# bertaveira/mojosplat

Measured on AMD Instinct MI355X. Metric: frames/sec at 1M Gaussians 1920x1080 fwd; achieved HBM GB/s vs peak, higher is better.
Workload: dtype f32

## Files before the change

### mojosplat_amd/csrc/binning.hip

```cpp
#include <hip/hip_fp16.h>
#include <stdlib.h>
#include <string.h>

#include <algorithm>
#include <atomic>
#include <mutex>
#include <type_traits>
#include <vector>

#include "project_device.hpp"

#ifdef MS_DIAG
__device__ unsigned long long *g_diag_bin = nullptr;
#define MS_BIN_STAMP(k, j) do { if (g_diag_bin && threadIdx.x == 0 && blockIdx.x < 1024) g_diag_bin[((k) * 1024 + blockIdx.x) * 8 + (j)] = __builtin_amdgcn_s_memrealtime(); } while (0)
#else
#define MS_BIN_STAMP(k, j) do { } while (0)
#endif

namespace {

#ifndef MS_CHUNK
#define MS_CHUNK 2048
#endif
#ifndef MS_PH_WAVES
#define MS_PH_WAVES 8
#endif
constexpr int kHistThreads = 1024;
#ifndef MS_CLAIM_GROUPS
#define MS_CLAIM_GROUPS 4
#endif
constexpr int kClaimGroups = MS_CLAIM_GROUPS;
constexpr int kClaimShift = kClaimGroups == 8 ? 0 : kClaimGroups == 4 ? 1 : kClaimGroups == 2 ? 2 : 3;
static_assert(kClaimGroups == 8 || kClaimGroups == 4 || kClaimGroups == 2 || kClaimGroups == 1, "claim groups: a power of two <= 8");
constexpr int kMaxG = 512;
constexpr int kSmallCapDecl = 1024, kMediumCapDecl = 8192, kLargeCapDecl = 16384;
constexpr int kCoopThreshold = 32;
constexpr int kBandCull = 32;
constexpr int kLightBucket = 32;
constexpr int kLightCap = 256;
constexpr int kLean = 64;
constexpr int kDeferTotal = 128;
static_assert(kLean == ms::kTightLean && kDeferTotal == ms::kTightDeferTotal, "internal flag bits out of sync");
constexpr size_t kMaxLds = 160 * 1024 - 4096;

struct Grid {
    int ts, tw, th, row_begin, row_end;
    int pack, cw, ch;
};

struct LeanRec {
    uint32_t xy0, xy1, depth_bits, n_edges;
};
struct Lean12 {
    uint32_t box, depth_bits, mask32;
};

__device__ __forceinline__ unsigned long long reach_mask(float mx, float my, float ca, float cb, float cc,
                                                        float opacity, int x0, int x1, int y0, int y1, int ts) {
    const int w = x1 - x0, h = y1 - y0;
    const float det = ca * cc - cb * cb;
    if (w * h > 64 || w * h <= 1 || !(det > 0.f) || !(ca > 0.f) || !(cc > 0.f) || !(opacity >= ms::kAlphaThreshold))
        return ~0ull;
    const float s2 = 2.0f * (__logf(opacity * 255.0f) * 1.0001f + 1e-4f);
    const float inv_det = __builtin_amdgcn_rcpf(det), inv_ca = __builtin_amdgcn_rcpf(ca);
    const float Y = __builtin_amdgcn_sqrtf(ca * s2 * inv_det);
    const float dy_right = -(cb * __builtin_amdgcn_rcpf(cc)) * __builtin_amdgcn_sqrtf(cc * s2 * inv_det);
    const float fts = (float)ts, span = (float)(ts - 1), inv_ts = __builtin_amdgcn_rcpf(fts);
    unsigned long long mask = 0;
    for (int r = 0; r < h; ++r) {
        const float yl = (float)((y0 + r) * ts) + 0.5f - my, yh = yl + span;
        const float lo = fmaxf(yl, -Y), hi = fminf(yh, Y);
        if (lo > hi + 0.01f) continue;
        const float dyr = fminf(fmaxf(dy_right, lo), hi), dyl = fminf(fmaxf(-dy_right, lo), hi);
        const float xmax = (-cb * dyr + __builtin_amdgcn_sqrtf(fmaxf(ca * s2 - det * dyr * dyr, 0.f))) * inv_ca + 0.01f;
        const float xmin = (-cb * dyl - __builtin_amdgcn_sqrtf(fmaxf(ca * s2 - det * dyl * dyl, 0.f))) * inv_ca - 0.01f;
        const float base = 0.5f - mx;
        int ta = (int)ceilf((xmin - base - span) * inv_ts - 1e-3f), tb = (int)floorf((xmax - base) * inv_ts + 1e-3f);
        ta = max(ta, x0); tb = min(tb, x1 - 1);
        if (ta > tb) continue;
        const unsigned long long rowbits = (tb - ta + 1 >= 64) ? ~0ull : ((1ull << (tb - ta + 1)) - 1ull);
        mask |= rowbits << (r * w + (ta - x0));
    }
    return mask;
}

__device__ __forceinline__ int chunk_of_block(int b, int G) {
    const int n8 = G >> 3, rem = G & 7, x = b & 7, k = b >> 3;
    return x * n8 + min(x, rem) + k;
}

#ifndef MS_DEAL
#define MS_DEAL 64
#endif
#ifndef MS_PH_TICKETS
#define MS_PH_TICKETS 1
#endif
constexpr int kDeal = MS_DEAL;
static_assert(kDeal >= 64 && kDeal <= 1024 && (kDeal & (kDeal - 1)) == 0, "a slice is a power-of-two number of waves");
struct Deal {
    int64_t n, first, stride;
    int iters;
    __device__ __forceinline__ Deal(int64_t n_pos, int wg, int G) {
        constexpr int kWavesPerSlice = kDeal / 64, kParts = kHistThreads / kDeal;
        const int w = __builtin_amdgcn_readfirstlane((int)(threadIdx.x >> 6));
        const int part = w / kWavesPerSlice, v = w - part * kWavesPerSlice;
        n = n_pos;
        first = ((int64_t)part * G + wg) * kDeal + (int64_t)v * 64;
        stride = (int64_t)kParts * G * kDeal;
        iters = (int)((n_pos + stride - 1) / stride);
    }
    __device__ __forceinline__ int64_t base(int it) const { return first + (int64_t)it * stride; }
};

__device__ __forceinline__ int clampi(float v, int lo, int hi) {
    if (!(v > (float)lo)) return lo;
    if (v >= (float)hi) return hi;
    return (int)v;
}

__device__ __forceinline__ bool tile_bbox(float2 m, int2 r, const Grid &g, int &x0, int &x1,
                                          int &y0, int &y1) {
    const float fts = (float)g.ts;
    float trx, try_, tx, ty;
    if ((g.ts & (g.ts - 1)) == 0) {
        const float inv = 1.0f / fts;
        trx = (float)r.x * inv; try_ = (float)r.y * inv;
        tx = m.x * inv; ty = m.y * inv;
    } else {
        trx = (float)r.x / fts; try_ = (float)r.y / fts;
        tx = m.x / fts; ty = m.y / fts;
    }
    x0 = clampi(floorf(tx - trx), 0, g.tw);
    x1 = clampi(ceilf(tx + trx), 0, g.tw);
    y0 = clampi(floorf(ty - try_), 0, g.th);
    y1 = clampi(ceilf(ty + try_), 0, g.th);
    const bool on_grid = x1 > x0 && y1 > y0;
    y0 = max(y0, g.row_begin);
    y1 = min(y1, g.row_end);
    y1 = max(y1, y0);
    return on_grid;
}

__device__ __forceinline__ void count_on_grid(bool on_grid, unsigned int *s_on_grid) {
    const unsigned long long b = __ballot(on_grid);
    if ((threadIdx.x & 63) == 0 && b) atomicAdd(s_on_grid, (unsigned int)__popcll(b));
}

template <bool PACK>
__device__ __forceinline__ bool bin_box(float2 m, int2 r, const Grid &g, int &x0, int &x1, int &y0, int &y1,
                                        int &edges) {
    edges = 0;
    if constexpr (!PACK) return tile_bbox(m, r, g, x0, x1, y0, y1);
    const Grid gc{g.ts >> 1, g.cw, g.ch, 0, g.ch, 0, 0, 0};
    int cx0, cx1, cy0, cy1;
    const bool on = tile_bbox(m, r, gc, cx0, cx1, cy0, cy1);
    x0 = cx0 >> 1; x1 = (cx1 + 1) >> 1;
    y0 = cy0 >> 1; y1 = (cy1 + 1) >> 1;
    if (!on) { x1 = x0; y1 = y0; }
    y0 = max(y0, g.row_begin);
    y1 = min(y1, g.row_end);
    y1 = max(y1, y0);
    edges = (cx0 > 2 * x0 ? 1 : 0) | (cx1 < 2 * x1 ? 2 : 0) | (cy0 > 2 * y0 ? 4 : 0) | (cy1 < 2 * y1 ? 8 : 0);
    return on;
}

__device__ __forceinline__ int edge_blocks(int edges, int c, int r, int w, int h) {
    int q = 0xf;
    if ((edges & 1) && c == 0) q &= 0xa;
    if ((edges & 2) && c == w - 1) q &= 0x5;
    if ((edges & 4) && r == 0) q &= 0xc;
    if ((edges & 8) && r == h - 1) q &= 0x3;
    return q;
}

__device__ __forceinline__ unsigned long long clip_cells(unsigned long long m, int edges, int w, int h) {
    const int cwid = 2 * w, rows = 2 * h;
    if (cwid * rows < 64) m &= (1ull << (cwid * rows)) - 1ull;
    if (edges & 4) m &= ~((1ull << cwid) - 1ull);
    if (edges & 8) m &= (1ull << ((rows - 1) * cwid)) - 1ull;
    if (edges & 3) {
        unsigned long long p = 1ull;
        for (int sh = cwid; sh < 64; sh <<= 1) p |= p << sh;
        if (edges & 1) m &= ~p;
        if (edges & 2) m &= ~(p << (cwid - 1));
    }
    return m;
}

struct BigQ {
    uint32_t *ent;
    unsigned int *count;
    unsigned int cap;
};

template <bool PACK, bool PAYLOAD, class F>
__device__ __forceinline__ void walk_boxes_impl(int gi, int x0, int x1, int y0, int y1, int n, int edges,
                                                const Grid &g, unsigned long long mask, F &&f, uint32_t payload,
                                                const BigQ *Q = nullptr) {
    auto call = [&](int t, int64_t i, int q, uint32_t pl) __attribute__((always_inline)) {
        if constexpr (PAYLOAD) f(t, i, q, pl);
        else f(t, i, q);
    };
    const int lane = threadIdx.x & 63;
    const int64_t i = gi;
    const bool big = n > kCoopThreshold;
    if (n > 0 && !big) {
        const int w = x1 - x0;
        const float inv_w = __builtin_amdgcn_rcpf((float)w);
        unsigned int m;
        const bool cells = PACK && n <= 16;
        if (cells) {
            const int cw = 2 * w, h = y1 - y0;
            const unsigned int rowmask = cw >= 32 ? 0xffffffffu : ((1u << cw) - 1u);
            m = 0;
            for (int r = 0; r < h; ++r) {
                unsigned int t = ((unsigned int)(mask >> (2 * r * cw)) | (unsigned int)(mask >> ((2 * r + 1) * cw))) & rowmask;
                t = (t | (t >> 1)) & 0x55555555u;
                t = (t | (t >> 1)) & 0x33333333u;
                t = (t | (t >> 2)) & 0x0f0f0f0fu;
                t = (t | (t >> 4)) & 0x00ff00ffu;
                t = (t | (t >> 8)) & 0x0000ffffu;
                m |= t << (r * w);
            }
        } else {
            m = (unsigned int)mask & (n >= 32 ? 0xffffffffu : ((1u << n) - 1u));
        }
        while (m) {
            const int k = __ffs((int)m) - 1;
            m &= m - 1;
            const int r = (int)(((float)k + 0.5f) * inv_w);
            const int c = k - r * w;
            int q;
            if (cells) {
                const int cw = 2 * w, b00 = 2 * r * cw + 2 * c;
                q = (int)((mask >> b00) & 3ull) | ((int)((mask >> (b00 + cw)) & 3ull) << 2);
            } else {
                q = PACK ? edge_blocks(edges, c, r, w, y1 - y0) : 0xf;
            }
            call((y0 + r - g.row_begin) * g.tw + x0 + c, i, q, payload);
        }
    }
    bool queued = false;
    if (Q && Q->cap && big) {
        const unsigned int slot = atomicAdd(Q->count, 1u);
        if (slot < Q->cap) {
            uint32_t *e = Q->ent + 8u * slot;
            e[0] = (uint32_t)x0 | ((uint32_t)y0 << 16); e[1] = (uint32_t)x1 | ((uint32_t)y1 << 16);
            e[2] = (uint32_t)gi; e[3] = payload;
            e[4] = (uint32_t)mask; e[5] = (uint32_t)(mask >> 32); e[6] = (uint32_t)edges;
            queued = true;
        }
    }
    unsigned long long bigmask = __ballot(big && !queued);
    while (bigmask) {
        const int src = __ffsll((long long)bigmask) - 1;
        bigmask &= bigmask - 1;
        const int bx0 = __builtin_amdgcn_readlane(x0, src), bx1 = __builtin_amdgcn_readlane(x1, src);
        const int by0 = __builtin_amdgcn_readlane(y0, src), by1 = __builtin_amdgcn_readlane(y1, src);
        const unsigned long long bm = ((unsigned long long)(unsigned)__builtin_amdgcn_readlane((int)(mask >> 32), src) << 32) |
                                      (unsigned)__builtin_amdgcn_readlane((int)(mask & 0xffffffffu), src);
        const int be = PACK ? __builtin_amdgcn_readlane(edges, src) : 0;
        const int64_t bi = __builtin_amdgcn_readlane(gi, src);
        const uint32_t bp = PAYLOAD ? (uint32_t)__builtin_amdgcn_readlane((int)payload, src) : 0u;
        const int w = bx1 - bx0, cnt = w * (by1 - by0);
        if (w <= 256 && cnt <= 65536) {
            const float inv_w = __builtin_amdgcn_rcpf((float)w);
            for (int k = lane; k < cnt; k += 64) {
                const int r = (int)(((float)k + 0.5f) * inv_w), c = k - r * w;
                if (cnt > 64 || ((bm >> k) & 1ull))
                    call((by0 + r - g.row_begin) * g.tw + bx0 + c, bi, PACK ? edge_blocks(be, c, r, w, by1 - by0) : 0xf, bp);
            }
        } else {
            for (int k = lane; k < cnt; k += 64) {
                const int r = k / w, c = k % w;
                call((by0 + r - g.row_begin) * g.tw + bx0 + c, bi, PACK ? edge_blocks(be, c, r, w, by1 - by0) : 0xf, bp);
            }
        }
    }
}

template <bool PACK, class F>
__device__ __forceinline__ void walk_boxes(int gi, int x0, int x1, int y0, int y1, int n, int edges,
                                           const Grid &g, unsigned long long mask, F &&f, const BigQ *Q = nullptr) {
    walk_boxes_impl<PACK, false>(gi, x0, x1, y0, y1, n, edges, g, mask, f, 0u, Q);
}
template <bool PACK, class F>
__device__ __forceinline__ void walk_boxes(int gi, int x0, int x1, int y0, int y1, int n, int edges,
                                           const Grid &g, unsigned long long mask, F &&f, uint32_t payload, const BigQ *Q = nullptr) {
    walk_boxes_impl<PACK, true>(gi, x0, x1, y0, y1, n, edges, g, mask, f, payload, Q);
}

template <bool PACK, bool PAYLOAD, class F>
__device__ __forceinline__ void drain_big_boxes(const BigQ &Q, const Grid &g, F &&f) {
    if (!Q.cap) return;
    __syncthreads();
    const unsigned int total = min(*Q.count, Q.cap);
    const int lane = threadIdx.x & 63;
    const unsigned int nw = blockDim.x >> 6;
    for (unsigned int e = (unsigned int)__builtin_amdgcn_readfirstlane((int)(threadIdx.x >> 6)); e < total; e += nw) {
        const uint32_t *q = Q.ent + 8u * e;
        const int bx0 = (int)(q[0] & 0xffffu), by0 = (int)(q[0] >> 16), bx1 = (int)(q[1] & 0xffffu), by1 = (int)(q[1] >> 16);
        const int64_t bi = (int64_t)(int32_t)q[2];
        const uint32_t bp = q[3];
        const unsigned long long bm = (unsigned long long)q[4] | ((unsigned long long)q[5] << 32);
        const int be = (int)q[6];
        const int w = bx1 - bx0, cnt = w * (by1 - by0);
        const float inv_w = __builtin_amdgcn_rcpf((float)max(w, 1));
        const bool by_rcp = w <= 256 && cnt <= 65536;
        for (int k = lane; k < cnt; k += 64) {
            const int r = by_rcp ? (int)(((float)k + 0.5f) * inv_w) : k / w, c = k - r * w;
            if (cnt > 64 || ((bm >> k) & 1ull)) {
                const int t = (by0 + r - g.row_begin) * g.tw + bx0 + c;
                const int qb = PACK ? edge_blocks(be, c, r, w, by1 - by0) : 0xf;
// ... 584 lines not shown
        const int t = tb + lane;
        unsigned int incl = c;
#pragma unroll
        for (int d = 1; d < 64; d <<= 1) {
            const unsigned int o = (unsigned int)__shfl_up((int)incl, d);
            if (lane >= d) incl += o;
        }
        if (t < w1) {
            const unsigned long long b = run + (incl - c), e = run + incl;
            reinterpret_cast<int2 *>(tile_ranges)[t] =
                make_int2((int32_t)min(b, 0x7fffffffull), (int32_t)min(e, 0x7fffffffull));
            redo_flag[t] = 0;
            lmax = max(lmax, c);
            if (c > (unsigned)kLargeCapDecl) xl_list[atomicAdd(&s_nxl, 1u)] = t;
            else if (c > (unsigned)kMediumCapDecl) large_list[atomicAdd(&s_nlarge, 1u)] = t;
            else if (c > (unsigned)kSmallCapDecl) medium_list[atomicAdd(&s_nmedium, 1u)] = t;
            if (order && t >= band0 && t < band1) atomicAdd(&s_bkt[bucket_of(c)], 1u);
        }
        run += (unsigned long long)__shfl((int)incl, 63);
    };
#pragma unroll
    for (int k = 0; k < kPre; ++k)
        if (w0 + k * 64 < w1) step(w0 + k * 64, pre[k]);
    for (int tb = w0 + kPre * 64; tb < w1; tb += 64) step(tb, count_of(tb + lane));
#pragma unroll
    for (int d = 32; d > 0; d >>= 1) lmax = max(lmax, (unsigned int)__shfl_xor((int)lmax, d));
    if (lane == 0) atomicMax(&s_max, lmax);
    __syncthreads();
    if (order) {
        if (w == 0) {
            const unsigned int c0 = s_bkt[127 - 2 * lane], c1 = s_bkt[126 - 2 * lane];
            unsigned int incl = c0 + c1;
#pragma unroll
            for (int d = 1; d < 64; d <<= 1) {
                const unsigned int o = (unsigned int)__shfl_up((int)incl, d);
                if (lane >= d) incl += o;
            }
            const unsigned int excl = incl - (c0 + c1);
            s_base[127 - 2 * lane] = excl;
            s_base[126 - 2 * lane] = excl + c0;
        }
        __syncthreads();
        if (threadIdx.x == 0 && A.wg_on_grid) const_cast<uint32_t *>(A.wg_on_grid)[kMaxG + 1] = s_base[kLightBucket];
        __syncthreads();
        auto place = [&](int t, unsigned int c) {
            if (t < w1 && t >= band0 && t < band1) order[atomicAdd(&s_base[bucket_of(c)], 1u)] = t;
        };
#pragma unroll
        for (int k = 0; k < kPre; ++k)
            if (w0 + k * 64 < w1) place(w0 + k * 64 + lane, pre[k]);
        for (int tb = w0 + kPre * 64; tb < w1; tb += 64) place(tb + lane, count_of(tb + lane));
    }
    if (threadIdx.x == 0) {
        info[0] = (int64_t)grand;
        info[1] = (int64_t)s_max;
        info[2] = (int64_t)s_nmedium;
        info[3] = (int64_t)s_nlarge;
        info[4] = (int64_t)s_nxl;
        {
            const int prev_cut = min(max(redo_count[1], 0), max(prev_redo, 0));
            info[5] = (int64_t)(prev_redo - prev_cut) + ((int64_t)(prev_cut & 0x3fffffff) << 32) + (prev_cut > 0 && info[10] != 0 ? (1ll << 62) : 0);
        }
        redo_count[0] = 0;
        redo_count[1] = 0;
        redo_count[2] = redo_signature(g);
        info[6] = (int64_t)s_on_grid;
        info[7] = 0;
        if (info_mirror) {
#pragma unroll
            for (int k = 0; k < 7; ++k) info_mirror[k] = info[k];
            __threadfence_system();
        }
    }
}

template <int kScanTiles>
__global__ __launch_bounds__(1024) void k_tile_scan_wg(int G, int T_local,
                                                       uint32_t *__restrict__ hist,
                                                       uint32_t *__restrict__ tile_count, ScanTotalArgs A) {
    constexpr int kScanSlices = 1024 / kScanTiles;
    __shared__ uint32_t s_part[16][kScanTiles];
    __shared__ int s_last;
    MS_BIN_STAMP(1, 0);
    const int lane = threadIdx.x & 63, w = threadIdx.x >> 6;
    const int tl = threadIdx.x & (kScanTiles - 1), sl = threadIdx.x / kScanTiles;
    const int t = blockIdx.x * kScanTiles + tl;
    constexpr int kRows = kMaxG / kScanSlices;
    const int per = (G + kScanSlices - 1) / kScanSlices;
    const int g0 = sl * per, g1 = min(G, g0 + per);
    uint32_t v[kRows];
    uint32_t sum = 0;
#pragma unroll
    for (int k = 0; k < kRows; ++k) {
        const int gg = g0 + k;
        v[k] = (k < per && gg < g1 && t < T_local) ? hist[(size_t)gg * T_local + t] : 0u;
        sum += v[k];
    }
    uint32_t incl = sum;
#pragma unroll
    for (int d = kScanTiles; d < 64; d <<= 1) {
        const uint32_t o = (uint32_t)__shfl_up((int)incl, d);
        if (lane >= d) incl += o;
    }
    if (lane >= 64 - kScanTiles) s_part[w][tl] = incl;
    MS_BIN_STAMP(1, 1);
    __syncthreads();
    MS_BIN_STAMP(1, 2);
    uint32_t run = incl - sum, total = 0;
#pragma unroll
    for (int ww = 0; ww < 16; ++ww) {
        const uint32_t p = s_part[ww][tl];
        if (ww < w) run += p;
        total += p;
    }
#pragma unroll
    for (int k = 0; k < kRows; ++k) {
        const int gg = g0 + k;
        if (k < per && gg < g1 && t < T_local) {
            hist[(size_t)gg * T_local + t] = run;
            run += v[k];
        }
    }
    if (!A.ticket) {
        if (sl == 0 && t < T_local) tile_count[t] = total;
        MS_BIN_STAMP(1, 3);
        return;
    }
    if (sl == 0 && t < T_local) __hip_atomic_store(&tile_count[t], total, __ATOMIC_RELAXED, __HIP_MEMORY_SCOPE_AGENT);
    asm volatile("s_waitcnt vmcnt(0)" ::: "memory");
    __builtin_amdgcn_fence(__ATOMIC_RELEASE, "workgroup");
    __syncthreads();
    if (threadIdx.x == 0) s_last = __hip_atomic_fetch_add(A.ticket, 1u, __ATOMIC_RELAXED, __HIP_MEMORY_SCOPE_AGENT) == gridDim.x - 1 ? 1 : 0;
    __syncthreads();
    if (!s_last) return;
    tile_scan_total<true>(A);
}

__global__ __launch_bounds__(1024) void k_tile_scan_total(ScanTotalArgs A) { tile_scan_total<false>(A); }

__device__ __forceinline__ unsigned long long tile_prefix_lds(const uint32_t *__restrict__ count, int T, uint32_t *s,
                                                              const uint32_t *__restrict__ add = nullptr,
                                                              const uint32_t *__restrict__ xtot = nullptr, int x_mine = 0) {
    __shared__ unsigned long long s_wtot[16];
    const int tid = threadIdx.x, lane = tid & 63, w = tid >> 6;
    const int per = (T + kHistThreads - 1) / kHistThreads;
    const int j0 = min(T, tid * per), j1 = min(T, j0 + per);
    uint32_t addv[4] = {0u, 0u, 0u, 0u};
    const bool pre = add && per <= 4;
    auto add_of = [&](int j) __attribute__((always_inline)) -> uint32_t {
        uint32_t v = add[j];
        if (xtot)
            for (int x = 0; x < x_mine; ++x) v += xtot[(size_t)x * T + j];
        return v;
    };
    if (pre) {
#pragma unroll
        for (int k = 0; k < 4; ++k)
            if (j0 + k < j1) addv[k] = add_of(j0 + k);
    }
    if (xtot) {
        for (int t = tid; t < T; t += kHistThreads) {
            uint32_t c = 0;
#pragma unroll
            for (int x = 0; x < kClaimGroups; ++x) c += xtot[(size_t)x * T + t];
            s[t] = c;
        }
    } else
    for (int t = tid; t < T; t += kHistThreads) s[t] = count[t];
    __syncthreads();
    unsigned long long sum = 0;
    for (int j = j0; j < j1; ++j) sum += s[j];
    unsigned long long incl = sum;
#pragma unroll
    for (int d = 1; d < 64; d <<= 1) {
        const unsigned long long o = __shfl_up(incl, d);
        if (lane >= d) incl += o;
    }
    if (lane == 63) s_wtot[w] = incl;
    __syncthreads();
    unsigned long long run = incl - sum, grand = 0;
#pragma unroll
    for (int ww = 0; ww < 16; ++ww) {
        if (ww < w) run += s_wtot[ww];
        grand += s_wtot[ww];
    }
    if (pre) {
#pragma unroll
        for (int k = 0; k < 4; ++k)
            if (j0 + k < j1) {
                const uint32_t v = s[j0 + k];
                s[j0 + k] = (uint32_t)min(run, 0x7fffffffull) + addv[k];
                run += v;
            }
    } else {
        for (int j = j0; j < j1; ++j) {
            const uint32_t v = s[j];
            s[j] = (uint32_t)min(run, 0x7fffffffull) + (add ? add_of(j) : 0u);
            run += v;
        }
    }
    __syncthreads();
    return grand;
}

__device__ __forceinline__ void deferred_total(int which, const ScanTotalArgs &A, uint32_t *s, int T_local) {
    const Grid &g = A.g;
    const int band0 = g.row_begin * g.tw, band1 = g.row_end * g.tw;
    const int tid = threadIdx.x, lane = tid & 63;
    if (which == 1) {
        if (!A.order) return;
        __shared__ unsigned int s_bkt[128], s_base[128];
        auto bucket_of = [](unsigned int c) -> int {
            if (c == 0) return 0;
            const int l = 31 - __clz((int)c);
            const int frac = l >= 2 ? (int)((c >> (l - 2)) & 3u) : (int)((c << (2 - l)) & 3u);
            return 1 + 4 * l + frac;
        };
        if (tid < 128) s_bkt[tid] = 0;
        __syncthreads();
        for (int t = tid; t < T_local; t += kHistThreads) atomicAdd(&s_bkt[bucket_of(tile_count_of(A, t, T_local))], 1u);
        __syncthreads();
        if (tid < 64) {
            const unsigned int c0 = s_bkt[127 - 2 * lane], c1 = s_bkt[126 - 2 * lane];
            unsigned int incl = c0 + c1;
#pragma unroll
            for (int d = 1; d < 64; d <<= 1) {
                const unsigned int o = (unsigned int)__shfl_up((int)incl, d);
                if (lane >= d) incl += o;
            }
            const unsigned int excl = incl - (c0 + c1);
            s_base[127 - 2 * lane] = excl;
            s_base[126 - 2 * lane] = excl + c0;
        }
        __syncthreads();
        if (tid == 0 && A.wg_on_grid) const_cast<uint32_t *>(A.wg_on_grid)[kMaxG + 1] = s_base[kLightBucket];
        __syncthreads();
        for (int t = tid; t < T_local; t += kHistThreads)
            A.order[atomicAdd(&s_base[bucket_of(tile_count_of(A, t, T_local))], 1u)] = band0 + t;
        return;
    }
    if (A.far_zero)
        for (int t = tid; t < 2 * A.g.tw * A.g.th; t += kHistThreads) A.far_zero[t] = 0u;
    __shared__ unsigned int s_nmedium, s_nlarge, s_nxl, s_max, s_on_grid, s_far;
    if (tid == 0) { s_nmedium = 0; s_nlarge = 0; s_nxl = 0; s_max = 0; s_on_grid = 0; s_far = 0; }
    const int prev_redo = (tid == 0 && A.redo_count[2] == redo_signature(A.g)) ? *A.redo_count : 0;
    unsigned int on_grid_part = tid < A.G ? A.wg_on_grid[tid] : 0u;
    unsigned int far_part = (A.wg_far && tid < A.G) ? A.wg_far[tid] : 0u;
    const unsigned long long grand = tile_prefix_lds(A.tile_count, T_local, s, nullptr, A.xtot);
    if (tid == 0) s[T_local] = (uint32_t)min(grand, 0x7fffffffull);
    __syncthreads();
#pragma unroll
    for (int d = 32; d > 0; d >>= 1) {
        on_grid_part += (unsigned int)__shfl_xor((int)on_grid_part, d);
        far_part += (unsigned int)__shfl_xor((int)far_part, d);
    }
    if (lane == 0 && on_grid_part) atomicAdd(&s_on_grid, on_grid_part);
    if (lane == 0 && far_part) atomicAdd(&s_far, far_part);
    unsigned int lmax = 0;
    for (int t = tid; t < T_local; t += kHistThreads) {
        const uint32_t b = s[t], e = s[t + 1], c = e - b;
        const int at = band0 + t;
        reinterpret_cast<int2 *>(A.tile_ranges)[at] = make_int2((int32_t)b, (int32_t)e);
        A.redo_flag[at] = 0;
        if (A.xtot) const_cast<uint32_t *>(A.tile_count)[t] = c;
        lmax = max(lmax, c);
        if (c > (unsigned)kLargeCapDecl) A.xl_list[atomicAdd(&s_nxl, 1u)] = at;
        else if (c > (unsigned)kMediumCapDecl) A.large_list[atomicAdd(&s_nlarge, 1u)] = at;
        else if (c > (unsigned)kSmallCapDecl) A.medium_list[atomicAdd(&s_nmedium, 1u)] = at;
    }
    if (!A.band_only) {
        const int32_t m = (int32_t)min(grand, 0x7fffffffull);
        for (int t = tid; t < g.tw * g.th; t += kHistThreads)
            if (t < band0 || t >= band1) {
                reinterpret_cast<int2 *>(A.tile_ranges)[t] = t < band0 ? make_int2(0, 0) : make_int2(m, m);
                A.redo_flag[t] = 0;
            }
    }
#pragma unroll
    for (int d = 32; d > 0; d >>= 1) lmax = max(lmax, (unsigned int)__shfl_xor((int)lmax, d));
    if (lane == 0) atomicMax(&s_max, lmax);
    __syncthreads();
    if (tid == 0) {
        const int prev_cut = min(max(A.redo_count[1], 0), max(prev_redo, 0));
        int64_t rec[7] = {(int64_t)grand + (int64_t)s_far, (int64_t)s_max, (int64_t)s_nmedium, (int64_t)s_nlarge, (int64_t)s_nxl,
                          (int64_t)(prev_redo - prev_cut) + ((int64_t)(prev_cut & 0x3fffffff) << 32) +
                              (prev_cut > 0 && A.info[10] != 0 ? (1ll << 62) : 0), (int64_t)s_on_grid};
#pragma unroll
        for (int k = 0; k < 7; ++k) A.info[k] = rec[k];
        A.info[7] = 0;
        A.info[8] = (int64_t)grand;
        A.info[9] = (int64_t)s_far;
        A.info[10] = 0;
        A.redo_count[0] = 0;
        A.redo_count[1] = 0;
        A.redo_count[2] = redo_signature(A.g);
        if (A.info_mirror) {
#pragma unroll
            for (int k = 0; k < 7; ++k) A.info_mirror[k] = rec[k];
            __threadfence_system();
        }
    }
}

#ifndef MS_SCATTER_WAVES
#define MS_SCATTER_WAVES 8
#endif
template <bool PACK, int LEAN, bool DEFER>
__global__ __launch_bounds__(kHistThreads, (LEAN == 2 ? MS_SCATTER_WAVES : 4)) void k_isect_scatter(
    int64_t N, const float *__restrict__ means2d, const int32_t *__restrict__ radii,
    const float *__restrict__ depths, const unsigned long long *__restrict__ masks,
    const LeanRec *__restrict__ lean, Grid g, int64_t chunk, const uint32_t *__restrict__ hist,
    const int32_t *__restrict__ tile_ranges, int64_t M, uint64_t *__restrict__ keys,
    uint32_t *__restrict__ wg_depth, Candidates cand, int G, ScanTotalArgs A, unsigned int big_q_off, unsigned int big_q_cap) {
    extern __shared__ uint32_t s_cur[];
    const int T_local = (g.row_end - g.row_begin) * g.tw;
    const int band0 = g.row_begin * g.tw;
    __shared__ unsigned int s_big_n;
    if (threadIdx.x == 0) s_big_n = 0;
    const BigQ bigq{reinterpret_cast<uint32_t *>(reinterpret_cast<char *>(s_cur) + big_q_off), &s_big_n, big_q_cap};
    MS_BIN_STAMP(2, 0);
    if constexpr (DEFER) {
        if ((int)blockIdx.x >= G) {
            deferred_total((int)blockIdx.x - G, A, s_cur, T_local);
            MS_BIN_STAMP(2, 4);
            return;
        }
    }
    const int wg = chunk_of_block(blockIdx.x, G);
    const uint32_t *row = hist + (size_t)wg * T_local;
    (void)chunk;
    int64_t n_pos = N;
    if constexpr (LEAN != 0) {
        if (cand.ids) {
            __shared__ uint32_t s_pref[kMaxG + 1];
            CandMap map{s_pref};
            map.build(cand);
            n_pos = (int64_t)s_pref[cand.n_segs];
        }
    }
    const Deal deal(n_pos, wg, G);
    constexpr int kAhead = 4;
    LeanRec r_q[kAhead], r_nx[kAhead];
    unsigned long long m_q[kAhead], m_nx[kAhead];
#pragma unroll
    for (int k = 0; k < kAhead; ++k) { r_q[k] = r_nx[k] = LeanRec{0u, 0u, 0u, 0u}; m_q[k] = m_nx[k] = ~0ull; }
    bool cut = false;
    if constexpr (LEAN == 2 && DEFER) cut = A.cut_stamp != 0u;
    int n_trips = deal.iters;
    int64_t cut_i0 = 0, cut_i1 = 0;
    if (cut) {
        cut_i0 = (int64_t)wg * A.near_cap;
        cut_i1 = cut_i0 + (int64_t)A.wg_far[kMaxG + wg];
        n_trips = (int)((cut_i1 - cut_i0 + kHistThreads - 1) / kHistThreads);
    }
    auto pos_of = [&](int it) __attribute__((always_inline)) -> int64_t {
        if (it >= n_trips) return -1;
        if (cut) {
            const int64_t j = cut_i0 + (int64_t)it * kHistThreads + threadIdx.x;
            return j < cut_i1 ? j : -1;
        }
        const int64_t j = deal.base(it) + (threadIdx.x & 63);
        return j < n_pos ? j : -1;
    };
    auto load_rec = [&](int64_t j, LeanRec &r, unsigned long long &m) __attribute__((always_inline)) {
        if constexpr (LEAN == 2) {
            if (cut) {
                r = A.near_recs[j];
            } else {
                const uint32_t *q = reinterpret_cast<const uint32_t *>(reinterpret_cast<const Lean12 *>(lean) + j);
                r.xy0 = q[0];
                r.xy1 = (uint32_t)j;
                r.depth_bits = q[1];
                r.n_edges = q[2];
            }
        } else {
            r = lean[j];
            if (masks) m = masks[j];
        }
    };
    auto unpack_rec = [&](LeanRec &r, unsigned long long &m, int64_t &gauss) __attribute__((always_inline)) {
        if constexpr (LEAN == 2) {
            const uint32_t box = r.xy0, mk = r.n_edges;
            gauss = (int64_t)r.xy1;
            const uint32_t x0 = box & 0xffu, y0 = (box >> 8) & 0xffu, w = (box >> 16) & 0xffu, h = box >> 24;
            r.xy0 = x0 | (y0 << 16);
            r.xy1 = (x0 + w) | ((y0 + h) << 16);
            r.n_edges = w * h;
            m = w * h > 32u ? ~0ull : (unsigned long long)mk;
        }
    };
    if constexpr (LEAN != 0) {
#pragma unroll
        for (int k = 0; k < kAhead; ++k) {
            const int64_t j = pos_of(k);
            if (j >= 0) load_rec(j, r_nx[k], m_nx[k]);
        }
    }
    MS_BIN_STAMP(2, 1);
    uint32_t *s_tau = s_cur + T_local + 4;
    if (cut)
        for (int t = threadIdx.x; t < T_local; t += kHistThreads) s_tau[t] = A.tau[band0 + t];
    if constexpr (DEFER) {
        (void)tile_prefix_lds(A.tile_count, T_local, s_cur, row, A.xtot, (int)(blockIdx.x & 7) >> kClaimShift);
        MS_BIN_STAMP(2, 2);
    } else {
        for (int t = threadIdx.x; t < T_local; t += kHistThreads) {
            uint32_t c = (uint32_t)tile_ranges[2 * (band0 + t)] + row[t];
            if (A.xtot)
                for (int x = 0; x < ((int)(blockIdx.x & 7) >> kClaimShift); ++x) c += A.xtot[(size_t)x * T_local + t];
            s_cur[t] = c;
        }
        __syncthreads();
    }
    uint32_t dmin = 0xffffffffu, dmax = 0u;
    if constexpr (LEAN != 0) {
        auto emit = [&](int t, int64_t i, int q, uint32_t db) __attribute__((always_inline)) {
            const uint32_t low = PACK ? (((uint32_t)i << 4) | (uint32_t)q) : (uint32_t)i;
            const uint64_t key = ((uint64_t)db << 32) | low;
            const uint32_t slot = atomicAdd(&s_cur[t], 1u);
            if ((int64_t)slot < M) keys[slot] = key;
        };
        auto emit_cut = [&](int t, int64_t i, int q, uint32_t db) __attribute__((always_inline)) { if (db <= s_tau[t]) emit(t, i, q, db); };
        for (int it0 = 0; it0 < n_trips; it0 += kAhead) {
#pragma unroll
            for (int k = 0; k < kAhead; ++k) { r_q[k] = r_nx[k]; m_q[k] = m_nx[k]; }
            if (it0 + kAhead < n_trips) {
#pragma unroll
                for (int k = 0; k < kAhead; ++k) {
                    const int64_t jn = pos_of(it0 + kAhead + k);
                    if (jn >= 0) load_rec(jn, r_nx[k], m_nx[k]);
                }
            }
#pragma unroll
            for (int k = 0; k < kAhead; ++k) {
                if (it0 + k >= n_trips) break;
                LeanRec r = r_q[k];
                unsigned long long mk = m_q[k];
                const int64_t j = pos_of(it0 + k);
                int64_t gi = j;
                unpack_rec(r, mk, gi);
                int x0 = 0, x1 = 0, y0 = 0, y1 = 0, n = 0, edges = 0;
                unsigned long long mask = ~0ull;
                if (j >= 0) {
                    n = (int)(r.n_edges & 0x0fffffffu);
                    edges = (int)(r.n_edges >> 28);
                    x0 = (int)(r.xy0 & 0xffffu); y0 = (int)(r.xy0 >> 16);
                    x1 = (int)(r.xy1 & 0xffffu); y1 = (int)(r.xy1 >> 16);
                    if (masks && (n > 1 || (PACK && n > 0) || cut)) mask = mk;
                }
                const uint32_t dbits = r.depth_bits;
                if (n > 0) { dmin = min(dmin, dbits); dmax = max(dmax, dbits); }
                if constexpr (!PACK) {
                    const int w = x1 - x0;
                    const float inv_w = __builtin_amdgcn_rcpf((float)max(w, 1));
                    unsigned int m = (n > 0 && n <= kCoopThreshold) ? ((unsigned int)mask & (n >= 32 ? 0xffffffffu : ((1u << n) - 1u))) : 0u;
                    const uint64_t key = ((uint64_t)dbits << 32) | (uint32_t)gi;
                    while (m) {
                        int tt[4];
                        bool vv[4];
                        uint32_t slot[4];
#pragma unroll
                        for (int u = 0; u < 4; ++u) {
                            vv[u] = m != 0u;
                            const int k = vv[u] ? __ffs((int)m) - 1 : 0;
                            m &= m - 1u;
                            const int r = (int)(((float)k + 0.5f) * inv_w);
                            tt[u] = (y0 + r - g.row_begin) * g.tw + x0 + (k - r * w);
                        }
#pragma unroll
                        for (int u = 0; u < 4; ++u)
                            if (vv[u]) slot[u] = atomicAdd(&s_cur[tt[u]], 1u);
#pragma unroll
                        for (int u = 0; u < 4; ++u)
                            if (vv[u] && (int64_t)slot[u] < M) keys[slot[u]] = key;
                    }
                    if (cut)
                        walk_boxes<PACK>((int)gi, x0, x1, y0, y1, n > kCoopThreshold ? n : 0, edges, g, mask, emit_cut, dbits, &bigq);
                    else
                        walk_boxes<PACK>((int)gi, x0, x1, y0, y1, n > kCoopThreshold ? n : 0, edges, g, mask, emit, dbits, &bigq);
                } else {
                    walk_boxes<PACK>((int)gi, x0, x1, y0, y1, n, edges, g, mask, emit, dbits, &bigq);
                }
            }
        }
        if (cut) drain_big_boxes<PACK, true>(bigq, g, emit_cut);
        else drain_big_boxes<PACK, true>(bigq, g, emit);
    } else {
        for_each_isect<PACK>(0, N, means2d, radii, masks, g, nullptr, nullptr, cand, G, [&](int t, int64_t i, int q) {
            const uint32_t slot = atomicAdd(&s_cur[t], 1u);
            const uint32_t low = PACK ? (((uint32_t)i << 4) | (uint32_t)q) : (uint32_t)i;
            const uint32_t dbits = __float_as_uint(depths[i]);
            dmin = min(dmin, dbits);
            dmax = max(dmax, dbits);
            const uint64_t key = ((uint64_t)dbits << 32) | low;
            if ((int64_t)slot < M) keys[slot] = key;
        });
    }
    MS_BIN_STAMP(2, 3);
#ifdef MS_DIAG
    if constexpr (LEAN != 0) { __syncthreads(); MS_BIN_STAMP(2, 4); }
#endif
    if (wg_depth) {
        uint32_t *s_depth = s_cur + T_local + 1;
        __syncthreads();
        if (threadIdx.x == 0) { s_depth[0] = 0xffffffffu; s_depth[1] = 0u; }
        __syncthreads();
#pragma unroll
        for (int d = 32; d > 0; d >>= 1) {
            dmin = min(dmin, (uint32_t)__shfl_xor((int)dmin, d));
            dmax = max(dmax, (uint32_t)__shfl_xor((int)dmax, d));
        }
        if ((threadIdx.x & 63) == 0) { atomicMin(&s_depth[0], dmin); atomicMax(&s_depth[1], dmax); }
        __syncthreads();
        if (threadIdx.x == 0) { wg_depth[2 * blockIdx.x] = s_depth[0]; wg_depth[2 * blockIdx.x + 1] = s_depth[1]; }
    }
}

}
#include "sort_device.hpp"
namespace {

constexpr int kSmallCap = SortCfg<256, 4>::CAP;
constexpr int kMediumCap = SortCfg<1024, 8>::CAP;
constexpr int kLargeCap = SortCfg<1024, 16>::CAP;

template <bool SPLIT>
__global__ __launch_bounds__(256) void k_tile_sort_small(const int32_t *__restrict__ tile_ranges,
                                                         const uint64_t *__restrict__ keys,
                                                         int32_t *__restrict__ flatten_ids,
                                                         int64_t *__restrict__ isect_ids, int64_t cap,
                                                         int tile_lo, ms::BlockLists blocks, int bin_w) {
    __shared__ __attribute__((aligned(16))) unsigned char smem[SortCfg<256, 4>::LDS];
    const int tile = tile_lo + blockIdx.x;
    const int start = tile_ranges[2 * tile], n = tile_ranges[2 * tile + 1] - start;
    const bool skip = n <= 0 || (int64_t)start + n > cap;
    if (SPLIT && (skip || n > kSmallCap)) {
        if (threadIdx.x < 4) {
            const int by = tile / bin_w, bx = tile - by * bin_w;
            const int x = 2 * bx + (threadIdx.x & 1), y = 2 * by + (threadIdx.x >> 1);
            if (x < blocks.tw16 && y < blocks.th16)
                reinterpret_cast<int2 *>(blocks.block_ranges)[y * blocks.tw16 + x] = make_int2(0, 0);
        }
        if (threadIdx.x == 0) blocks.bin_more[tile] = 0;
    }
    if (skip || n > kSmallCap) return;
    sort_segment_lds<256, 4>(smem, keys, start, n, tile, flatten_ids, isect_ids, nullptr, SPLIT ? &blocks : nullptr,
                             bin_w);
}

template <int E>
__global__ __launch_bounds__(1024, (E <= 8 ? 8 : 4)) void k_tile_sort_list(const int32_t *__restrict__ list,
                                                         const int32_t *__restrict__ tile_ranges,
                                                         const uint64_t *__restrict__ keys,
                                                         int32_t *__restrict__ flatten_ids,
                                                         int64_t *__restrict__ isect_ids,
                                                         const int64_t *__restrict__ n_list_dev,
                                                         int n_list_host, int64_t cap) {
    extern __shared__ __attribute__((aligned(16))) unsigned char smem_dyn[];
    const int n_list = n_list_dev ? (int)*n_list_dev : n_list_host;
    for (int li = blockIdx.x; li < n_list; li += gridDim.x) {
        const int tile = list[li];
        const int start = tile_ranges[2 * tile], n = tile_ranges[2 * tile + 1] - start;
        if ((int64_t)start + n <= cap)
            sort_segment_lds<1024, E>(smem_dyn, keys, start, n, tile, flatten_ids, isect_ids, nullptr);
        __syncthreads();
    }
}

#ifndef MS_MERGED_WAVES
#define MS_MERGED_WAVES 6
#endif
constexpr int kFrontThreads = 512;
static_assert(kFrontNB == 4 * kFrontThreads, "four buckets per thread in the scan");
constexpr size_t kFrontLds = (size_t)kFrontCap * 8 + (size_t)kFrontNB * 4 + 64 * 4 + 16;

template <bool SPLIT, bool MERGED>
__global__ __launch_bounds__(kFrontThreads, (MERGED ? MS_MERGED_WAVES : 1)) void k_tile_front(const int32_t *__restrict__ medium,
                                                     const int32_t *__restrict__ large,
                                                     const int32_t *__restrict__ xl,
                                                     const int64_t *__restrict__ info_dev, int nm_host, int nl_host,
                                                     int nx_host, const int32_t *__restrict__ tile_ranges,
                                                     const uint64_t *__restrict__ keys,
                                                     int32_t *__restrict__ flatten_ids,
                                                     int32_t *__restrict__ front_count, int64_t cap,
                                                     uint32_t fixed_min, int fixed_shift, int front_k,
                                                     ms::BlockLists blocks, int bin_w,
                                                     const uint32_t *__restrict__ wg_depth, int n_wg,
                                                     const int32_t *__restrict__ order, int n_order, int front_cap,
                                                     const uint32_t *__restrict__ n_big_dev,
                                                     uint32_t *__restrict__ tau, const uint32_t *__restrict__ tau_now,
                                                     const uint32_t *__restrict__ has_far, uint32_t cut_stamp) {
    static_assert(!(SPLIT && MERGED), "block lists are cut by the two-launch path");
    auto next_cut_whole = [&](int tile) {
        if (tau) tau[tile] = (cut_stamp && has_far[tile] == cut_stamp) ? tau_now[tile] : 0xffffffffu;
    };
    extern __shared__ __attribute__((aligned(16))) unsigned char smem_dyn[];
    uint64_t *s_out = reinterpret_cast<uint64_t *>(smem_dyn);
    uint32_t *s_cnt = reinterpret_cast<uint32_t *>(s_out + front_cap);
    uint32_t *s_red = s_cnt + kFrontNB;
    int *s_sel = reinterpret_cast<int *>(s_red + 64);
    constexpr int THREADS = kFrontThreads, NW = kFrontThreads / 64;
    const int tid = threadIdx.x, lane = tid & 63, w = tid >> 6;
    const int nm = info_dev ? (int)info_dev[2] : nm_host, nl = info_dev ? (int)info_dev[3] : nl_host;
    const int nx = info_dev ? (int)info_dev[4] : nx_host;
    const int total = MERGED ? n_order : nm + nl + nx;
    if ((int)blockIdx.x >= total) return;
    const int n_big = (MERGED && n_big_dev) ? min((int)*n_big_dev, total) : -1;
    if constexpr (MERGED) {
        if (n_big >= 0 && (int)blockIdx.x >= n_big) {
            const int e = n_big + 8 * ((int)blockIdx.x - n_big) + w;
            if (e < total) {
                const int tile = order[e];
                const int start = tile_ranges[2 * tile], n = tile_ranges[2 * tile + 1] - start;
                if (n > 0 && n <= kLightCap && (int64_t)start + n <= cap)
                    sort_segment_lds<64, kLightCap / 64>(smem_dyn + (size_t)w * SortCfg<64, kLightCap / 64>::LDS, keys, start, n, tile,
                                                         flatten_ids, nullptr, nullptr);
                if (lane == 0) next_cut_whole(tile);
            }
            return;
        }
    }
#ifdef MS_DIAG
    if (g_diag_bin && tid == 0) g_diag_bin[(3 * 1024 + (blockIdx.x & 1023)) * 8 + (blockIdx.x >> 10) * 3] = __builtin_amdgcn_s_memrealtime();
#endif
    bool range_known = false;
    auto frame_range = [&]() {
      if (wg_depth && !range_known) {
        uint32_t lo = 0xffffffffu, hi = 0u;
        for (int j = tid; j < n_wg; j += THREADS) {
            lo = min(lo, wg_depth[2 * j]);
            hi = max(hi, wg_depth[2 * j + 1]);
        }
#pragma unroll
        for (int d = 32; d > 0; d >>= 1) {
            lo = min(lo, (uint32_t)__shfl_xor((int)lo, d));
            hi = max(hi, (uint32_t)__shfl_xor((int)hi, d));
        }
        if (lane == 0) { s_red[w] = lo; s_red[16 + w] = hi; }
        __syncthreads();
#pragma unroll
        for (int ww = 0; ww < NW; ++ww) { lo = min(lo, s_red[ww]); hi = max(hi, s_red[16 + ww]); }
        __syncthreads();
        if (hi >= lo) {
            const uint32_t span = hi - lo;
            const int bits = span ? 32 - __clz(span) : 0;
            fixed_min = lo;
            fixed_shift = max(0, bits - kFrontLogNB);
        }
      }
      range_known = true;
    };
    if constexpr (!MERGED) frame_range();
    for (int li = blockIdx.x; li < total; li += gridDim.x) {
        const int tile = MERGED ? order[li] : li < nm ? medium[li] : (li < nm + nl ? large[li - nm] : xl[li - nm - nl]);
        const int start = tile_ranges[2 * tile], n = tile_ranges[2 * tile + 1] - start;
        if constexpr (MERGED) {
            if (n <= kSmallCap) {
                if (n > 0 && (int64_t)start + n <= cap)
                    sort_segment_lds<kFrontThreads, kSmallCap / kFrontThreads>(smem_dyn, keys, start, n, tile, flatten_ids,
                                                                               nullptr, nullptr);
                if (tid == 0) next_cut_whole(tile);
                __syncthreads();
#ifdef MS_DIAG
                if (g_diag_bin && tid == 0) {
                    unsigned long long *d = g_diag_bin + (3 * 1024 + (blockIdx.x & 1023)) * 8 + (blockIdx.x >> 10) * 3;
                    d[1] = __builtin_amdgcn_s_memrealtime(); d[2] = (unsigned long long)n;
                }
#endif
                continue;
            }
            frame_range();
        }
        if ((int64_t)start + n > cap) {
            if (SPLIT) {
                if (tid < 4) {
                    const int by = tile / bin_w, bx = tile - by * bin_w;
                    const int x = 2 * bx + (tid & 1), y = 2 * by + (tid >> 1);
                    if (x < blocks.tw16 && y < blocks.th16)
                        reinterpret_cast<int2 *>(blocks.block_ranges)[y * blocks.tw16 + x] = make_int2(0, 0);
                }
                if (tid == 0) blocks.bin_more[tile] = 0;
            }
            continue;
        }
        const int F = front_select_lds<THREADS, (SPLIT ? 8 : 4)>(keys + start, n, s_out, s_cnt, s_red, s_sel, fixed_min, fixed_shift,
                                                                 front_k, front_cap);
        if constexpr (SPLIT) emit_block_lists<THREADS, kFrontCap / THREADS>(s_out, F, n, start, tile, bin_w, blocks, s_cnt);
        else
            for (int i = tid; i < F; i += THREADS) flatten_ids[start + i] = (int32_t)(uint32_t)s_out[i];
        if (tid == 0) front_count[tile] = F;
        if (MERGED && tid == 0 && tau) {
            if (F >= n) next_cut_whole(tile);
            else {
                const uint32_t edge = (uint32_t)s_sel[2];
                const unsigned long long cut = (unsigned long long)edge + (1ull << 19);
                tau[tile] = (uint32_t)(cut > 0xffffffffull ? 0xffffffffull : cut);
            }
        }
        __syncthreads();
#ifdef MS_DIAG
        if (g_diag_bin && tid == 0) {
            unsigned long long *d = g_diag_bin + (3 * 1024 + (blockIdx.x & 1023)) * 8 + (blockIdx.x >> 10) * 3;
            d[1] = __builtin_amdgcn_s_memrealtime(); d[2] = (unsigned long long)n;
        }
#endif
    }
}

__global__ __launch_bounds__(1024) void k_xl_chunk_sort(const int32_t *__restrict__ xl_list,
                                                        const int32_t *__restrict__ tile_ranges,
                                                        uint64_t *__restrict__ keys) {
    extern __shared__ __attribute__((aligned(16))) unsigned char smem_dyn[];
    const int tile = xl_list[blockIdx.y];
    const int start = tile_ranges[2 * tile], n = tile_ranges[2 * tile + 1] - start;
    const int c0 = blockIdx.x * kLargeCap;
    if (c0 >= n) return;
    const int cn = min(kLargeCap, n - c0);
    sort_segment_lds<1024, 16>(smem_dyn, keys, start + c0, cn, tile, nullptr, nullptr, keys);
}

__global__ __launch_bounds__(256) void k_xl_merge(const int32_t *__restrict__ xl_list,
                                                  const int32_t *__restrict__ tile_ranges,
                                                  const uint64_t *__restrict__ src,
                                                  uint64_t *__restrict__ dst, int L) {
    const int tile = xl_list[blockIdx.y];
    const int start = tile_ranges[2 * tile], n = tile_ranges[2 * tile + 1] - start;
    const int e = blockIdx.x * 256 + threadIdx.x;
    if (e >= n) return;
    const uint64_t key = src[start + e];
    const int run = e / L, pos = e - run * L;
    const int pair_base = (run & ~1) * L;
    const int pb = (run ^ 1) * L;
    int cnt = 0;
    if (pb < n) {
        const int pn = min(L, n - pb);
        int lo = 0, hi = pn;
        const uint64_t *p = src + start + pb;
        while (lo < hi) {
            const int mid = (lo + hi) >> 1;
            if (p[mid] < key) lo = mid + 1; else hi = mid;
        }
        cnt = lo;
    }
    dst[start + pair_base + pos + cnt] = key;
}

__global__ __launch_bounds__(256) void k_xl_extract(const int32_t *__restrict__ xl_list,
                                                    const int32_t *__restrict__ tile_ranges,
                                                    const uint64_t *__restrict__ src,
                                                    int32_t *__restrict__ flatten_ids,
                                                    int64_t *__restrict__ isect_ids) {
    const int tile = xl_list[blockIdx.y];
    const int start = tile_ranges[2 * tile], n = tile_ranges[2 * tile + 1] - start;
    const int e = blockIdx.x * 256 + threadIdx.x;
    if (e >= n) return;
    const uint64_t k = src[start + e];
    flatten_ids[start + e] = (int32_t)(uint32_t)k;
    if (isect_ids) isect_ids[start + e] = ((int64_t)tile << 32) | (int64_t)(k >> 32);
}

__global__ __launch_bounds__(256) void k_offset_encode(int64_t M, const int64_t *__restrict__ ids,
                                                       int T, int32_t *__restrict__ offsets) {
    const int64_t idx = (int64_t)blockIdx.x * 256 + threadIdx.x;
    if (idx >= M) return;
    const int cur = (int)(ids[idx] >> 32);
    if (idx == 0)
        for (int t = 0; t <= cur && t < T; ++t) offsets[t] = 0;
    else {
        const int prev = (int)(ids[idx - 1] >> 32);
        for (int t = prev + 1; t <= cur && t < T; ++t) offsets[t] = (int32_t)idx;
    }
    if (idx == M - 1)
        for (int t = cur + 1; t < T; ++t) offsets[t] = (int32_t)M;
}

struct Plan {
    int G;
    int64_t chunk;
    int64_t near_cap;
    int T, T_local;
    size_t lds_bytes;
    size_t off_xtot;
// ... 867 lines not shown
```

Measured before the change: 6244.

## Load-balance small-box scatter across wave lanes via prefix-sum expansion

```diff
diff --git a/mojosplat_amd/csrc/binning.hip b/mojosplat_amd/csrc/binning.hip
--- a/mojosplat_amd/csrc/binning.hip
+++ b/mojosplat_amd/csrc/binning.hip
@@ -9,6 +9,7 @@
 #include <vector>
 
 #include "project_device.hpp"
+#include "scatter_expand.hpp"
 
 #ifdef MS_DIAG
 __device__ unsigned long long *g_diag_bin = nullptr;
@@ -1199,6 +1200,17 @@
     }
 }
 
+__device__ __forceinline__ uint32_t wave_prefix_add(uint32_t v) {
+    int x = (int)v;
+    x += __builtin_amdgcn_update_dpp(0, x, 0x111, 0xf, 0xf, false);
+    x += __builtin_amdgcn_update_dpp(0, x, 0x112, 0xf, 0xf, false);
+    x += __builtin_amdgcn_update_dpp(0, x, 0x114, 0xf, 0xf, false);
+    x += __builtin_amdgcn_update_dpp(0, x, 0x118, 0xf, 0xf, false);
+    x += __builtin_amdgcn_update_dpp(0, x, 0x142, 0xa, 0xf, false);
+    x += __builtin_amdgcn_update_dpp(0, x, 0x143, 0xc, 0xf, false);
+    return (uint32_t)x;
+}
+
 #ifndef MS_SCATTER_WAVES
 #define MS_SCATTER_WAVES 8
 #endif
@@ -1348,33 +1360,46 @@
                 const uint32_t dbits = r.depth_bits;
                 if (n > 0) { dmin = min(dmin, dbits); dmax = max(dmax, dbits); }
                 if constexpr (!PACK) {
+                    const unsigned int m = (n > 0 && n <= kCoopThreshold) ? ((unsigned int)mask & (n >= 32 ? 0xffffffffu : ((1u << n) - 1u))) : 0u;
                     const int w = x1 - x0;
-                    const float inv_w = __builtin_amdgcn_rcpf((float)max(w, 1));
-                    unsigned int m = (n > 0 && n <= kCoopThreshold) ? ((unsigned int)mask & (n >= 32 ? 0xffffffffu : ((1u << n) - 1u))) : 0u;
-                    const uint64_t key = ((uint64_t)dbits << 32) | (uint32_t)gi;
-                    while (m) {
-                        int tt[4];
-                        bool vv[4];
-                        uint32_t slot[4];
-#pragma unroll
-                        for (int u = 0; u < 4; ++u) {
-                            vv[u] = m != 0u;
-                            const int k = vv[u] ? __ffs((int)m) - 1 : 0;
-                            m &= m - 1u;
-                            const int r = (int)(((float)k + 0.5f) * inv_w);
-                            tt[u] = (y0 + r - g.row_begin) * g.tw + x0 + (k - r * w);
-                        }
-#pragma unroll
-                        for (int u = 0; u < 4; ++u)
-                            if (vv[u]) slot[u] = atomicAdd(&s_cur[tt[u]], 1u);
-#pragma unroll
-                        for (int u = 0; u < 4; ++u)
-                            if (vv[u] && (int64_t)slot[u] < M) keys[slot[u]] = key;
-                    }
+                    const uint32_t geo = LEAN == 2 ? ((uint32_t)x0 | ((uint32_t)w << 8) | ((uint32_t)y0 << 16)) : ((uint32_t)x0 | ((uint32_t)y0 << 16));
                     if (cut)
                         walk_boxes<PACK>((int)gi, x0, x1, y0, y1, n > kCoopThreshold ? n : 0, edges, g, mask, emit_cut, dbits, &bigq);
                     else
                         walk_boxes<PACK>((int)gi, x0, x1, y0, y1, n > kCoopThreshold ? n : 0, edges, g, mask, emit, dbits, &bigq);
+                    const int ln = (int)(threadIdx.x & 63);
+                    const uint32_t incl = wave_prefix_add((uint32_t)__popc(m));
+                    const uint32_t total = (uint32_t)__builtin_amdgcn_readlane((int)incl, 63);
+                    uint32_t grp[7];
+#pragma unroll
+                    for (int j = 0; j < 7; ++j) grp[j] = (uint32_t)__builtin_amdgcn_readlane((int)incl, 8 * j + 7);
+                    for (uint32_t base = 0; base < total; base += 64u) {
+                        const uint32_t p = base + (uint32_t)ln;
+                        int owner;
+                        uint32_t rank;
+                        ms_expand::owner_rank<6, 3>(p, [&](int j) __attribute__((always_inline)) { return grp[j]; },
+                                                    [&](int i) __attribute__((always_inline)) {
+                            return (uint32_t)__builtin_amdgcn_ds_bpermute(i << 2, (int)incl); }, owner, rank);
+                        const uint32_t om = (uint32_t)__builtin_amdgcn_ds_bpermute(owner << 2, (int)m);
+                        const uint32_t og = (uint32_t)__builtin_amdgcn_ds_bpermute(owner << 2, (int)geo);
+                        int ow, ox0, oy0;
+                        if constexpr (LEAN == 2) {
+                            ox0 = (int)(og & 0xffu); ow = (int)((og >> 8) & 0xffu); oy0 = (int)(og >> 16);
+                        } else {
+                            ox0 = (int)(og & 0xffffu); oy0 = (int)(og >> 16);
+                            ow = __builtin_amdgcn_ds_bpermute(owner << 2, w);
+                        }
+                        const bool live = p < total;
+                        const int k = ms_expand::kth_set_bit(om, live ? rank : 0u);
+                        const float inv_w = __builtin_amdgcn_rcpf((float)max(ow, 1));
+                        const int r = (int)(((float)k + 0.5f) * inv_w);
+                        const int t = (oy0 + r - g.row_begin) * g.tw + ox0 + (k - r * ow);
+                        uint32_t slot = 0xffffffffu;
+                        if (live) slot = atomicAdd(&s_cur[t], 1u);
+                        const uint32_t od = (uint32_t)__builtin_amdgcn_ds_bpermute(owner << 2, (int)dbits);
+                        const uint32_t oi = (uint32_t)__builtin_amdgcn_ds_bpermute(owner << 2, (int)(uint32_t)gi);
+                        if (live && (int64_t)slot < M) keys[slot] = ((uint64_t)od << 32) | oi;
+                    }
                 } else {
                     walk_boxes<PACK>((int)gi, x0, x1, y0, y1, n, edges, g, mask, emit, dbits, &bigq);
                 }
diff --git a/mojosplat_amd/csrc/scatter_expand.hpp b/mojosplat_amd/csrc/scatter_expand.hpp
--- /dev/null
+++ b/mojosplat_amd/csrc/scatter_expand.hpp
@@ -0,0 +1,54 @@
+#pragma once
+#include <cstdint>
+
+#if defined(__HIPCC__) || defined(__CUDACC__)
+#define MS_EXPAND_HD __host__ __device__ __forceinline__
+#else
+#define MS_EXPAND_HD inline
+#endif
+
+namespace ms_expand {
+
+MS_EXPAND_HD int kth_set_bit(uint32_t m, uint32_t k) {
+    int pos = 0;
+#define MS_EXPAND_STEP(W, MASK)                                            \
+    {                                                                      \
+        const uint32_t c = (uint32_t)__builtin_popcount(m & (MASK));       \
+        const bool up = k >= c;                                            \
+        k -= up ? c : 0u;                                                  \
+        m = up ? (m >> (W)) : m;                                           \
+        pos += up ? (W) : 0;                                               \
+    }
+    MS_EXPAND_STEP(16, 0xffffu)
+    MS_EXPAND_STEP(8, 0xffu)
+    MS_EXPAND_STEP(4, 0xfu)
+    MS_EXPAND_STEP(2, 0x3u)
+    MS_EXPAND_STEP(1, 0x1u)
+#undef MS_EXPAND_STEP
+    return pos;
+}
+
+template <int LOG2N, int LOG2C, class Coarse, class Probe>
+MS_EXPAND_HD void owner_rank(uint32_t p, Coarse &&coarse_at, Probe &&incl_at, int &owner, uint32_t &rank) {
+    static_assert(LOG2C >= 0 && LOG2C <= LOG2N, "group size");
+    int lo = 0;
+    uint32_t excl = 0u;
+#pragma unroll
+    for (int j = 0; j < (1 << (LOG2N - LOG2C)) - 1; ++j) {
+        const uint32_t v = coarse_at(j);
+        const bool up = v <= p;
+        lo += up ? (1 << LOG2C) : 0;
+        excl = up ? v : excl;
+    }
+#pragma unroll
+    for (int step = (1 << LOG2C) >> 1; step > 0; step >>= 1) {
+        const uint32_t v = incl_at(lo + step - 1);
+        const bool up = v <= p;
+        lo += up ? step : 0;
+        excl = up ? v : excl;
+    }
+    owner = lo;
+    rank = p - excl;
+}
+
+}
```

After: 6288, median of 6. About the same (+0.7%).
